# NathanBWaters/playaid_core

Hardware: AMD Instinct MI355X
Metric: 1080p frames/sec end-to-end (higher is better)
Workload: dtype f32; 1 GPU; configs[1]: 64 x 1080x1920 BGR frames per GPU per clip; parallelism=single GPU, lanes=2, ingest=raw BGR frames resident in HBM

## Files before the change

playaid_core_amd/csrc/igemm.hip:

```cpp
#include "tile_common.h"
#include <cstdio>
#include <cstdlib>

namespace pa {

#ifndef PA_COUNTED_VMCNT
#define PA_COUNTED_VMCNT 0
#endif

template <int BM, int BN, int BK, bool GATHER, int ABL = 0, bool SKIPW = false>
__global__ __launch_bounds__(256) void igemm_f32_kernel(const GemmParams p) {
    constexpr int MI = BM / 64;
    constexpr int NI = BN / 64;
    using Stage = Im2colStage<4, BK, BM, BN, GATHER>;
    constexpr int LDS_STRIDE = BK;
    constexpr int A_ROWS = Stage::A_ROWS, B_ROWS = Stage::B_ROWS;
    constexpr int STAGE = (BM + BN) * LDS_STRIDE;
    __shared__ __attribute__((aligned(16))) float lds[3 * STAGE];

    Stage st;
    st.setup(p);
    const int tile_m = st.tile_m, tile_n = st.tile_n, z = st.z;
    const int ks_begin = st.ks_begin, ks_end = st.ks_end;
    const int tid = threadIdx.x;
    const int wave_id = __builtin_amdgcn_readfirstlane(tid >> 6);
#define PA_ISSUE_STAGE(BUF)                                                \
    {                                                                      \
        float* As_w = lds + (BUF) * STAGE + wave_id * 256;                 \
        st.issue(p, As_w, As_w + BM * LDS_STRIDE);                         \
    }

    const int lane = tid & 63;
    const int wave = tid >> 6;
    const int wm = wave >> 1, wn = wave & 1;
    const int lr = lane & 31;
    const int lh = lane >> 5;
// ... 222 lines not shown
    plan_splitk(p.ktot / bk, p.splitk, p.ksteps_per_split);
    hipError_t err;
    switch (tile) {
        case TILE_128x128: err = launch_tile<128, 128, 32>(p, s); break;
        case TILE_128x64: err = launch_tile<128, 64, 32>(p, s); break;
        case TILE_64x64: err = launch_tile<64, 64, 32>(p, s); break;
        case TILE_128x64_K64: err = launch_tile<128, 64, 64>(p, s); break;
        default: err = launch_tile<64, 64, 64>(p, s); break;
    }
    if (err != hipSuccess) return err;
    if (p.splitk_used) *p.splitk_used = p.splitk;
    if (p.splitk > 1 && !p.defer_reduce) return launch_splitk_reduce(p, s);
    return hipSuccess;
}

hipError_t launch_splitk_reduce(const GemmParams& p, hipStream_t s, bool out_bf16) {
    const size_t total = (size_t)p.M * (p.N >> 2);
    int grid = (int)((total + 255) / 256);
    if (grid > 2048) grid = 2048;
    if (out_bf16) hipLaunchKernelGGL(splitk_reduce_kernel<bf16_t>, dim3(grid), dim3(256), 0, s, p);
    else hipLaunchKernelGGL(splitk_reduce_kernel<float>, dim3(grid), dim3(256), 0, s, p);
    return hipGetLastError();
}

}
```

playaid_core_amd/csrc/misc.hip:

```cpp
#include "tile_common.h"
#include "../../include/playaid_hip.h"

namespace pa {

__global__ __launch_bounds__(256) void nchw_to_padded_kernel(const float* __restrict__ x, float* __restrict__ out, int n, int out_bf16) {
    const size_t total = (size_t)n * 128 * 128;
    for (size_t i = (size_t)blockIdx.x * blockDim.x + threadIdx.x; i < total; i += (size_t)gridDim.x * blockDim.x) {
        const int img = (int)(i >> 14);
        const int pix = (int)(i & 16383);
        const int y = pix >> 7, xx = pix & 127;
        const float* s = x + (size_t)img * 3 * 16384 + pix;
        float4 v;
        v.x = s[0];
        v.y = s[16384];
        v.z = s[32768];
        v.w = 0.f;
        const size_t o = ((size_t)img * 134 + (y + 3)) * 134 + (xx + 3);
        if (out_bf16) {
            reinterpret_cast<uint2*>(out)[o] = make_uint2(pack_bf16x2(v.x, v.y), f32_to_bf16(v.z));
        } else {
            reinterpret_cast<float4*>(out)[o] = v;
        }
    }
}
// ... 115 lines not shown
        sum.x *= 0.0625f;
        sum.y *= 0.0625f;
        sum.z *= 0.0625f;
        sum.w *= 0.0625f;
        reinterpret_cast<float4*>(out)[i] = sum;
    }
}

hipError_t launch_avgpool(const float* in, float* out, int32_t n, hipStream_t s) {
    const size_t total = (size_t)n * 128;
    const int grid = (int)((total + 255) / 256);
    hipLaunchKernelGGL(avgpool_kernel, dim3(grid), dim3(256), 0, s, in, out, n);
    return hipGetLastError();
}

__global__ void window_gather_kernel(int32_t* gather, int frame_num_lo, int count, int fighters, int seq, int delta,
                                     int max_frames, int min_frame, int sub_frames) {
    const int i = blockIdx.x * blockDim.x + threadIdx.x;
    const int total = count * fighters * seq;
    if (i >= total) return;
    const int t = i % seq;
    const int w = i / seq;
    const int fighter = w % fighters;
    const int f = frame_num_lo + w / fighters;
    if (sub_frames > 0) {
        const int c = (f - 1) / sub_frames;
        min_frame = c * sub_frames + 1;
        max_frames = (c + 1) * sub_frames;
    }
    const int mid = seq / 2;
// ... 182 lines not shown
```

playaid_core_amd/csrc/pa_api.hip:

```cpp
#include "../../include/playaid_hip.h"
#include "conv_rows.h"

#include <algorithm>
#include <cmath>
#include <cstdio>
#include <cstdlib>
#include <cstring>
#include <string>
#include <vector>

using namespace pa;

namespace {

constexpr int WINO_TICKETS = 4096;

struct ConvLayer {
    std::string name;
    int cin, cout, kh, kw, stride;
    int in_hw, out_hw;
    int in_pad, out_pad;
    int off;
    int taps, kw_taps, chunk;
    int in_px_stride;
// ... 3 lines not shown
    float* wgt = nullptr;
    float* wino_wgt = nullptr;
    int wino_bn = 0;
    float* bias = nullptr;
    int relu = 1;
    GemmTile tile = TILE_128x64;
    int splitk = 1;
    bool forced = false;
    float* in2 = nullptr;
    int in2_c = 0, in2_hw = 0, in2_stride = 1;
    float* ds_wgt = nullptr;
    float* ds_out = nullptr;
    float* ds_next_wgt = nullptr;
    float* ds_next_out = nullptr;
    std::string ds_next_name;
    bool ds_fused = false;
    bool ds_probe = false;
    double k_alg = 0;
    unsigned short* split_wgt = nullptr;
    unsigned short* ds_split_wgt = nullptr;
};

struct ProfEntry {
    int name_id;
    hipEvent_t start, stop;
    double flops, bytes;
    double flops_executed;
};

}
// ... 24 lines not shown
    float* x0 = nullptr;
    float* x0_slot[2] = {nullptr, nullptr};
    int32_t* pre_status[2] = {nullptr, nullptr};
    float* pooled = nullptr;
    float* feats_tmp = nullptr;
    float* cache = nullptr;
    int32_t* cache_status = nullptr;
    float* h1 = nullptr;
    int32_t* gather = nullptr;
    int gather_key[4] = {-1, -1, -1, -1};
    float* slab = nullptr;
    size_t slab_floats = 0;
    float* wino_tickets = nullptr;
    std::vector<ConvLayer> convs;
    ConvLayer fc;
    float* stem_wgt_bf16 = nullptr;
    float* c1 = nullptr;
    float* p1 = nullptr;
    float* layer4_out = nullptr;
    float* w1d = nullptr;
    float* b1d = nullptr;
    float *w2 = nullptr, *b2 = nullptr, *w3 = nullptr, *b3 = nullptr;
    GemmTile head_tile = TILE_64x64;
    int head_splitk = 16;
    CropPlan* plans = nullptr;
    int32_t* coef = nullptr;
    int coef_dim = 0;
    int32_t* coef_cache = nullptr;
    int coef_cache_pad = -1, coef_cache_dmax = 0;
    AreaTabPacked* area_tabs = nullptr;
// ... 275 lines not shown
        p.k2_steps = L.in2_c / (bf ? 64 : 32);
        p.in2_px_stride = L.in2_c;
        p.in2_row_stride = w2 * L.in2_c;
        p.in2_img_stride = w2 * w2 * L.in2_c;
        p.stride2 = L.in2_stride;
        p.off2 = 1;
        p.ktot += L.in2_c;
    }
    GemmTile tile = L.tile;
    int splitk = L.splitk;
    if (!L.forced) choose_tile(p.M, p.N, p.ktot / (bf ? 64 : 32), &tile, &splitk);
    p.splitk = splitk;
    const size_t slab_avail = e->slab_floats > slab_off ? e->slab_floats - slab_off : 0;
    if ((size_t)p.splitk * p.M * p.N > slab_avail) p.splitk = 1;
    const bool f32_branch = !bf && !e->emu && L.ds_next_wgt;
    const bool f32_branch_here = f32_branch && p.splitk <= 1;
    const bool ds_here = (bf && L.ds_next_wgt) || f32_branch_here;
    if (bf && L.ds_next_wgt) {
        p.wgt2 = L.ds_next_wgt;
        p.out2 = at(L.ds_next_out, crop0 * out_crop);
    }
    if ((bf && L.ds_next_wgt) || (bf && L.ds_probe)) {
        tile = (p.N % 128 == 0 && ((p.M + 127) / 128) * (p.N / 128) >= 256) ? TILE_128x128 : TILE_128x64;
        p.splitk = 1;
    }
    const double k_main = ((bf_ds || f32_ds) ? L.k_alg - L.in2_c : L.k_alg) + (ds_here ? L.cin : 0);
    const double flops = 2.0 * p.M * p.N * k_main;
    const double bytes = (double)es * ((double)ncrops * L.in_hw * L.in_hw * L.cin + (double)p.M * p.N * ((L.residual || bf_ds || f32_ds || ds_here) ? 2 : 1) +
                                       (double)p.N * k_main + ((L.in2 && !bf_ds && !f32_ds) ? (double)ncrops * L.in2_hw * L.in2_hw * L.in2_c : 0.0));
    const bool as_wino = !bf && L.wino_wgt && !p.act2;
    bool branch_left = f32_branch;
    {
// ... 29 lines not shown
            if (pe == hipErrorInvalidValue) pe = launch_igemm(p, tile, s);
            HIPCHK(e, pe);
        } else {
            static const int use_pgemm = getenv("PA_S2_PGEMM") ? atoi(getenv("PA_S2_PGEMM")) : 2;
            hipError_t pe = hipErrorInvalidValue;
            const bool pg = use_pgemm && L.kh == 3 && L.stride == 2 && !p.act2 && !p.residual && p.splitk <= 1 && !p.gather;
            if (pg && f32_branch_here) {
                p.wgt2 = L.ds_next_wgt;
                p.out2 = at(L.ds_next_out, crop0 * out_crop);
                pe = launch_pgemm(p, 64, s);
                if (pe == hipSuccess) branch_left = false;
                p.wgt2 = nullptr;
                p.out2 = nullptr;
            }
            if (pg && pe == hipErrorInvalidValue) pe = launch_pgemm(p, use_pgemm == 2 ? 64 : 0, s);
            if (pe == hipErrorInvalidValue) pe = launch_igemm(p, tile, s);
            HIPCHK(e, pe);
        }
    }
    if (branch_left) {
        const GemmParams d = branch_gemm_of(L.in, L.in_hw, L.cin, L.stride, L.ds_next_wgt, L.ds_next_out);
        ProfScope ps(e, s, e->profile_layers ? L.ds_next_name.c_str() : prof_name, 2.0 * d.M * d.N * L.cin,
                     4.0 * ((double)ncrops * L.in_hw * L.in_hw * L.cin / (L.stride * L.stride) + (double)d.M * d.N + (double)d.N * L.cin));
        HIPCHK(e, launch_f32_branch(d));
    }
    return PA_OK;
}

int run_backbone_part(pa_engine* e, int crop0, int ncrops, const float* x_in, float* feats_out, size_t slab_off, hipStream_t s,
                      int stop = PA_TRACE_STAGES) {
    int rc;
    ConvLayer stem = e->convs[0];
    stem.in = const_cast<float*>(x_in);
    static const bool stem_igemm = getenv("PA_STEM_IGEMM") && atoi(getenv("PA_STEM_IGEMM"));
    auto stem_part = [&](int c0, int n, hipStream_t st) -> int {
        if (stem_igemm && !e->bf16) return run_conv(e, stem, c0, n, slab_off, st, "igemm_conv7x7_stem");
        StemParams sp;
        memset(&sp, 0, sizeof(sp));
        sp.x = x_in + (size_t)c0 * 134 * 134 * 4;
// ... 62 lines not shown
                if ((rc = run_conv(e, Nx, crop0, ncrops, slab_off, e->side, "igemm_conv1x1_ds", true))) return rc;
                HIPCHK(e, hipEventRecord(e->ev_ds_join, e->side));
                ds_pending = true;
            }
        }
        const bool use_pending = ds_pending && L.in2 && L.ds_wgt && L.wino_wgt;
        if (use_pending) HIPCHK(e, hipStreamWaitEvent(s, e->ev_ds_join, 0));
        rc = run_conv(e, L, crop0, ncrops, slab_off, s, pn, false, use_pending);
        if (use_pending) ds_pending = false;
        if (rc) return rc;
        if (stop <= (int)i + 1) {
            if (ds_pending) HIPCHK(e, hipStreamWaitEvent(s, e->ev_ds_join, 0));
            return PA_OK;
        }
    }
    {
        ProfScope ps(e, s, "avgpool", 0.0, ncrops * ((e->bf16 ? 2.0 : 4.0) * 16.0 * 512 + 4.0 * 512));
        if (e->bf16)
            HIPCHK(e, launch_avgpool_bf16(reinterpret_cast<uint16_t*>(e->layer4_out) + (size_t)crop0 * 36 * 512,
                                          e->pooled + (size_t)crop0 * 512, ncrops, s));
        else
            HIPCHK(e, launch_avgpool(e->layer4_out + (size_t)crop0 * 36 * 512, e->pooled + (size_t)crop0 * 512, ncrops, s));
    }
    if (stop <= 18) return PA_OK;
    ConvLayer fc = e->fc;
    fc.out = feats_out;
    rc = run_conv(e, fc, crop0, ncrops, slab_off, s, "igemm_fc");
    return rc;
}

// ... 202 lines not shown
    ALLOC(e->c1, (size_t)NC * 66 * 66 * 64, true);
    ALLOC(e->p1, (size_t)NC * 34 * 34 * 64, true);
    ALLOC(e->pooled, (size_t)NC * 512, true);
    ALLOC(e->feats_tmp, (size_t)NC * PA_FEATURE_STRIDE, true);
    ALLOC(e->jpeg_qtab, 128, true);
    ALLOC(e->crops_tmp, (size_t)NC * PA_CROP * PA_CROP * 3, true);
    ALLOC(e->cache, (size_t)e->cache_rows * PA_FEATURE_STRIDE, true);
    ALLOC(e->cache_status, (size_t)e->cache_rows, true);
    ALLOC(e->h1, (size_t)NC * 512, true);
    ALLOC(e->gather, (size_t)NC * S, true);
    ALLOC(e->status_tmp, (size_t)NC, true);
    ALLOC(e->dev_errors, 4, true);
    e->clean_g6_cap = (size_t)cfg->max_clip_frames * 8 * 6;
    ALLOC(e->clean_g6, e->clean_g6_cap, false);

    e->arena_cap = pa_weight_blob_bytes(S, A) / 4 * 13 + (1u << 20);
    {
        void* ar = nullptr;
        HIPCHK(e, hipMalloc(&ar, e->arena_cap));
        e->allocs.push_back(ar);
        e->arena = reinterpret_cast<uint8_t*>(ar);
    }
    if (!e->adopt) e->arena_stage.assign(e->arena_cap, 0);
    static const float dry_source[1] = {0.f};
    const float* blob_f = e->adopt ? dry_source : reinterpret_cast<const float*>(hdr + 8);
    BlobReader br{blob_f, 0, blob_float_count(S, A), e->adopt};
    std::vector<float> keep_w, keep_b;
    auto add_conv = [&](const std::string& name, int cin, int cout, int k, int stride, int in_hw, float* in, float* outb,
                        float* residual, int relu, bool keep = false) -> int {
        ConvLayer L;
        L.name = name;
// ... 115 lines not shown
                    static const int wino_min_hw = getenv("PA_WINO_MIN_HW") ? atoi(getenv("PA_WINO_MIN_HW")) : 4;
                    if (wino_mode && wino_ds && hw_out >= wino_min_hw && hw_out % 4 == 0) {
                        L.wino_bn = wino_pick_bn(co, (long long)NC * (hw_out / 4) * (hw_out / 4), co);
                        std::vector<float> ug(wino_weight_floats(co, co), 0.f);
                        if (!br.dry) wino_transform_weights(keep_w.data(), co, co, L.wino_bn, ug.data());
                        rc = upload(e, &L.wino_wgt, ug);
                        if (rc) return rc;
                        rc = upload(e, &L.ds_wgt, wd);
                        if (rc) return rc;
                        if (e->emu && (rc = upload_split(e, &L.ds_split_wgt, wd, co, cin, false))) return rc;
                        ALLOC(L.ds_out, buf, true);
                        static const int f32_ds_fuse = getenv("PA_F32_DS_FUSE") ? atoi(getenv("PA_F32_DS_FUSE")) : 1;
                        static const int ds_side_knob = getenv("PA_DS_SIDE") ? atoi(getenv("PA_DS_SIDE")) : 0;
                        static const int s2_pgemm_knob = getenv("PA_S2_PGEMM") ? atoi(getenv("PA_S2_PGEMM")) : 2;
                        ConvLayer& C1 = e->convs[e->convs.size() - 2];
                        if (f32_ds_fuse && !ds_side_knob && s2_pgemm_knob && !e->emu && li < 3 && C1.in == cur && C1.kh == 3 &&
                            C1.stride == 2 && C1.cout == co && C1.out_hw == hw_out && C1.out_pad == L.out_pad && C1.chunk == cin && C1.cin == cin &&
                            C1.in_hw == hw_in[li] && C1.in_pad == 1 && !C1.forced) {
                            C1.ds_next_wgt = L.ds_wgt;
                            C1.ds_next_out = L.ds_out;
                            C1.ds_next_name = L.name;
                            L.ds_fused = true;
                        }
                    }
                }
                rc = upload(e, &L.bias, bf);
                if (rc) return rc;
                L.in2 = cur;
                L.in2_c = cin;
                L.in2_hw = hw_in[li];
                L.in2_stride = stride;
                L.k_alg += cin;
            }
            rc = add_conv(pre + ".1.conv1", co, co, 3, 1, hw_out, outA, mid, nullptr, 1);
            if (rc) return rc;
            rc = add_conv(pre + ".1.conv2", co, co, 3, 1, hw_out, mid, outB, outA, 1);
// ... 11 lines not shown
        if (!br.dry) {
            memcpy(wp.data(), w, sizeof(float) * 1000 * 512);
            memcpy(bp.data(), b, sizeof(float) * 1000);
        }
        ConvLayer& L = e->fc;
        L.name = "fc";
        L.cin = 512; L.cout = PA_FEATURE_STRIDE; L.kh = L.kw = 1; L.stride = 1;
        L.in_hw = 1; L.out_hw = 1; L.in_pad = 0; L.out_pad = 0; L.off = 0;
        L.taps = 1; L.kw_taps = 1; L.chunk = 512; L.in_px_stride = 512;
        L.in = e->pooled; L.out = nullptr; L.residual = nullptr; L.relu = 0;
        L.k_alg = 512.0 * 1000.0 / 1024.0;
        rc = upload(e, &L.wgt, wp);
        if (rc) return rc;
        rc = upload(e, &L.bias, bp);
        if (rc) return rc;
        L.tile = TILE_64x64;
        L.splitk = 4;
        L.forced = true;
        if (const char* fs = getenv("PA_FC_SPLITK")) L.splitk = std::max(1, atoi(fs));
    }
    {
        const float* w = br.take((size_t)512 * 1000 * S);
        const float* b = br.take(512);
        if (!w || !b) return fail(e, PA_ERR_BAD_WEIGHTS, "weight blob too short at cnn1d");
        std::vector<float> wp((size_t)512 * S * PA_FEATURE_STRIDE, 0.f);
        for (int o = 0; o < 512 && !br.dry; ++o)
            for (int c = 0; c < 1000; ++c)
                for (int t = 0; t < S; ++t)
                    wp[((size_t)o * S + t) * PA_FEATURE_STRIDE + c] = w[((size_t)o * 1000 + c) * S + t];
        rc = upload(e, &e->w1d, wp);
// ... 169 lines not shown
        bytes = n * w * w * L.cout * es;
        has_branch = L.in2 != nullptr;
        aux_src = L.ds_out;
    } else if (stage == 18) {
        src = e->pooled;
        bytes = n * 512 * sizeof(float);
    } else {
        src = e->feats_tmp;
        bytes = n * PA_FEATURE_STRIDE * sizeof(float);
    }
    if (out_bytes < bytes) return fail(e, PA_ERR_INVALID_ARG, "pa_backbone_trace: out is smaller than the stage");
    if (has_branch && aux) {
        if (!aux_src) return fail(e, PA_ERR_INVALID_ARG, "pa_backbone_trace: this stage stores no downsample branch");
        if (aux_bytes < bytes) return fail(e, PA_ERR_INVALID_ARG, "pa_backbone_trace: aux is smaller than the stage");
    }
    hipStream_t s = (hipStream_t)stream;
    HIPCHK(e, launch_nchw_to_padded(x, e->x0, n_crops, e->bf16 ? 1 : 0, s));
    if (stage > 0) {
        const int rc = run_backbone(e, n_crops, e->x0, e->feats_tmp, s, stage);
        if (rc) return rc;
    }
    HIPCHK(e, hipMemcpyAsync(out, src, bytes, hipMemcpyDeviceToDevice, s));
    if (has_branch && aux) HIPCHK(e, hipMemcpyAsync(aux, aux_src, bytes, hipMemcpyDeviceToDevice, s));
    return PA_OK;
}

int pa_crop_resize_width(pa_engine* e, const uint8_t* frames, int32_t n, int32_t height, int32_t width, const int32_t* rects_host,
                         int32_t n_rects, int32_t out_w, uint8_t* out, int32_t out_h_cap, int32_t* out_h_host, void* stream) {
    if (!e || !frames || !rects_host || !out || !out_h_host || n < 1 || height < 1 || width < 1 || n_rects < 1 || n_rects > 4 || out_w < 1 ||
        out_h_cap < 1)
        return fail(e, PA_ERR_INVALID_ARG, "pa_crop_resize_width: bad argument");
    RectResizeParams q;
    memset(&q, 0, sizeof(q));
    q.frames = frames;
    q.height = height;
    q.width = width;
    q.n_rects = n_rects;
    q.out_w = out_w;
// ... 248 lines not shown
    hipStream_t s = (hipStream_t)stream;
    const int F = e->cfg.num_fighters;
    HIPCHK(e, hipMemcpyAsync(e->cache_status + (size_t)frame0 * F, e->pre_status[slot], sizeof(int32_t) * n * F,
                             hipMemcpyDeviceToDevice, s));
    int rc = run_backbone(e, n * F, e->x0_slot[slot], e->cache + (size_t)frame0 * F * PA_FEATURE_STRIDE, s);
    if (rc) return rc;
    for (int i = 0; i < n; ++i) e->ready[frame0 + i] = 1;
    return PA_OK;
}

int pa_backbone_frames(pa_engine* e, const uint8_t* frames, int32_t n, int32_t height, int32_t width, const double* boxes,
                       int32_t frame0, uint8_t* crops_rgb, int32_t* status, void* stream) {
    if (!e || frame0 < 0) return fail(e, PA_ERR_INVALID_ARG, "pa_backbone_frames: bad argument");
    if (e->clip_frames < 1) return fail(e, PA_ERR_INVALID_ARG, "pa_backbone_frames: call pa_clip_begin first");
    if (frame0 + n > e->clip_frames) return fail(e, PA_ERR_CAPACITY, "pa_backbone_frames: frames exceed clip capacity");
    int rc = pa_preprocess_frames(e, frames, n, height, width, boxes, 0, crops_rgb, status, stream);
    if (rc) return rc;
    return pa_backbone_slot(e, 0, n, frame0, stream);
}

int pa_backbone_frames_indexed(pa_engine* e, const uint8_t* frames, int32_t n, int32_t height, int32_t width,
                               const double* boxes, const int32_t* frame_ids, uint8_t* crops_rgb, int32_t* status, void* stream) {
    if (!e || !frame_ids) return fail(e, PA_ERR_INVALID_ARG, "pa_backbone_frames_indexed: bad argument");
    if (e->clip_frames < 1) return fail(e, PA_ERR_INVALID_ARG, "pa_backbone_frames_indexed: call pa_clip_begin first");
    int rc = pa_preprocess_frames(e, frames, n, height, width, boxes, 0, crops_rgb, status, stream);
    if (rc) return rc;
    hipStream_t s = (hipStream_t)stream;
    const int F = e->cfg.num_fighters;
    rc = run_backbone(e, n * F, e->x0_slot[0], e->feats_tmp, s);
    if (rc) return rc;
    ProfScope ps(e, s, "scatter_features", 0.0, 2.0 * n * F * PA_FEATURE_STRIDE * 4.0);
    HIPCHK(e, launch_scatter_rows(e->feats_tmp, e->pre_status[0], frame_ids, e->cache, e->cache_status, n, F, e->clip_frames,
                                  e->dev_errors, s));
// ... 472 lines not shown
```

playaid_core_amd/csrc/pa_kernels.h:

```cpp
#pragma once
#include <hip/hip_runtime.h>
#include <stdint.h>

namespace pa {

__device__ __forceinline__ float silu_fast(float x) {
    return x * __builtin_amdgcn_rcpf(1.0f + __builtin_amdgcn_exp2f(x * -1.44269504088896341f));
}

struct GemmParams {
    const float* act;
    const float* wgt;
    const float* bias;
    const float* residual;
    float* out;
    float* slab;
    const int32_t* gather;
    int32_t M, N, ktot;
    int32_t taps, kw_taps, chunk;
    int32_t howo, wo;
    int32_t howo_shift, wo_shift;
    int32_t in_img_stride, in_row_stride, in_px_stride, stride, off_y, off_x;
    int32_t out_img_stride, out_row_stride, out_px_stride, out_pad;
    int32_t relu;
// ... 11 lines not shown
    int32_t up_img_stride, up_row_stride, up_px_stride, up_pad;
    int32_t patch_slots, patch_pitch, img_px, tiles_per_img, p0_img, p0_row, total_px;
    int32_t swz_a, magic_pitch, magic_img, img_px_patch;
    int32_t xcd_m, xcd_n;
    int32_t blk_rows, blk_cols, blk_shift_c, blk_shift_px, blk_per_row, blk_per_img, n_blocks, src_pitch;
    const float* wgt2;
    float* out2;
    unsigned long long* clk;
    int32_t* tickets;
};

enum GemmTile { TILE_128x128 = 0, TILE_128x64 = 1, TILE_64x64 = 2, TILE_128x64_K64 = 3, TILE_64x64_K64 = 4,
                TILE_256x128 = 5  };

hipError_t launch_igemm(const GemmParams& p, GemmTile tile, hipStream_t s);
hipError_t launch_pgemm(const GemmParams& p, int bm, hipStream_t s);
int psgemm_pick_bn(int N, int residual);
size_t psgemm_weight_elems(int N, int ktot, int residual);
void psgemm_pack_weights(const float* w, int N, int ktot, int residual, unsigned short* out);
hipError_t launch_psgemm(const GemmParams& p, const unsigned short* wsp, size_t out_floats, size_t up_floats, hipStream_t s);
size_t bgemm_weight_elems(int N, int ktot, int residual);
void bgemm_pack_weights(const float* w, int N, int ktot, int residual, unsigned short* out);
hipError_t launch_bgemm(const GemmParams& p, const unsigned short* wsp, size_t out_elems, size_t up_elems, bool out_f32, hipStream_t s);
constexpr int BGEMM_SLAB_ITEMS = 256, BGEMM_TICKETS = 4 * 128, BGEMM_SPLIT_MAX_GRID = 64, BGEMM_SPLIT_MIN_KSTEPS = 72;
int bgemm_pick_split(const GemmParams& p, int force);
hipError_t launch_igemm_bf16(const GemmParams& p, GemmTile tile, hipStream_t s);

hipError_t launch_conv3x3_bf16_patch(const GemmParams& p, hipStream_t s);

struct StemParams {
// ... 210 lines not shown
    float img_w, img_h;
    float* dets;
    int32_t* counts;
};
hipError_t launch_detect_nms(const DetectParams& q, hipStream_t s);
constexpr int DETECT_MAX_CLASSES = 80;
hipError_t launch_detect_nms_classes(const DetectParams& q, hipStream_t s);

hipError_t launch_linear_f32(const float* X, int ld, const float* W, const float* bias, float* C, int ldc, int M, int N, int K, int relu,
                             hipStream_t s);
hipError_t launch_spin(int32_t microseconds, hipStream_t s);
hipError_t launch_gate(const int* flag, int32_t max_microseconds, hipStream_t s);
hipError_t launch_nchw_to_padded(const float* x, float* out, int32_t n, int32_t out_bf16, hipStream_t s);
hipError_t launch_maxpool(const float* in, float* out, int32_t n, hipStream_t s);
hipError_t launch_avgpool(const float* in, float* out, int32_t n, hipStream_t s);
hipError_t launch_maxpool_bf16(const void* in, void* out, int32_t n, hipStream_t s);
hipError_t launch_avgpool_bf16(const void* in, float* out, int32_t n, hipStream_t s);
hipError_t launch_window_gather(int32_t* gather, int32_t frame_num_lo, int32_t count, int32_t fighters,
                                int32_t seq, int32_t delta, int32_t max_frames, int32_t min_frame, int32_t sub_frames, hipStream_t s);
hipError_t launch_identity_gather(int32_t* gather, int32_t n, hipStream_t s);
hipError_t launch_scatter_rows(const float* feats, const int32_t* st, const int32_t* ids, float* cache, int32_t* cache_st,
                               int32_t n, int32_t fighters, int32_t clip_frames, int32_t* bad_ids, hipStream_t s);

struct HeadParams {
    const float* h1;
    const float* slab;
    const float* b1;
    int32_t splitk;
    const float* w2;
    const float* b2;
// ... 29 lines not shown
```

playaid_core_amd/csrc/tile_common.h:

```cpp
#pragma once
#include "pa_kernels.h"

namespace pa {


typedef float f32x16 __attribute__((ext_vector_type(16)));
typedef float f32x4 __attribute__((ext_vector_type(4)));
typedef float f32x2 __attribute__((ext_vector_type(2)));
typedef uint32_t u32x4 __attribute__((ext_vector_type(4)));
typedef __bf16 bf16x8 __attribute__((ext_vector_type(8)));
typedef uint16_t bf16_t;

__device__ __forceinline__ int xcd_remap(int b, int nwg) {
    const int q = nwg >> 3, r = nwg & 7, xcd = b & 7;
    return (xcd < r ? xcd * (q + 1) : r * (q + 1) + (xcd - r) * q) + (b >> 3);
}

__device__ __forceinline__ void xcd_grid_tile(int xcd, int rank, int gm, int gn, int tiles_m, int tiles_n, int& tile_m, int& tile_n) {
    const int tm_per = tiles_m / gm, tn_per = tiles_n / gn;
    const int xm = xcd / gn, lm = rank / tn_per;
    tile_m = xm * tm_per + lm;
    tile_n = (xcd - xm * gn) * tn_per + (rank - lm * tn_per);
}

// ... 55 lines not shown
struct Im2colStage {
    static constexpr int CH = BK * EB / 16;
    static constexpr int PASS_ROWS = 256 / CH;
    static constexpr int A_ROWS = BM / PASS_ROWS;
    static constexpr int B_ROWS = BN / PASS_ROWS;
    static constexpr int CE = 16 / EB;

    int z, tile_m, tile_n;
    int row0, colq;
    int a_off[A_ROWS], a_off2[A_ROWS], b_off[B_ROWS];
    int nk_main, ks_begin, ks_end;
    int issue_ks;
    int cur_kc, cur_kx, cur_ky;
    __amdgpu_buffer_rsrc_t act_rs, wgt_rs, act2_rs;

    __device__ __forceinline__ void setup(const GemmParams& p) {
        const int wg = xcd_remap(blockIdx.x, gridDim.x);
        const int tiles_mn = p.tiles_m * p.tiles_n;
        z = wg / tiles_mn;
        const int t_id = wg - z * tiles_mn;
        tile_m = t_id / p.tiles_n;
        tile_n = t_id - tile_m * p.tiles_n;

        const int tid = threadIdx.x;
        row0 = tid / CH;
        colq = (tid & (CH - 1)) ^ (CH == 8 ? ((row0 >> 1) & 7) : (row0 & 15));
#pragma unroll
        for (int i = 0; i < A_ROWS; ++i) {
            int m = tile_m * BM + row0 + PASS_ROWS * i;
            m = m < p.M ? m : p.M - 1;
            a_off2[i] = 0;
            if (GATHER) {
// ... 124 lines not shown
```

playaid_core_amd/engine.py:

```python
from __future__ import annotations

import ctypes as C
from typing import Dict, List, Mapping, Optional, Tuple

import numpy as np
import torch

from . import _lib, constants
from .weights import infer_geometry, pack_state_dict


class EngineError(RuntimeError):
    def __init__(self, code: int, msg: str):
        super().__init__(f"playaid_hip error {code}: {msg}")
        self.code = code


def _ptr(t: Optional[torch.Tensor]):
    return C.c_void_p(t.data_ptr()) if t is not None else C.c_void_p(0)


class WeightsArena:

    def __init__(self, data: torch.Tensor, sequence_length: int, num_actions: int, compute_dtype: str):
# ... 153 lines not shown
        if stage == 1:
            return (n, 34, 34, 64)
        if 2 <= stage <= 17:
            li = (stage - 2) // 4
            hw = (32, 16, 8, 4)[li] + 2
            return (n, hw, hw, (64, 128, 256, 512)[li])
        if stage == 18:
            return (n, 512)
        if stage == 19:
            return (n, _lib.PA_FEATURE_STRIDE)
        raise ValueError(f"stage must be 0..{_lib.PA_TRACE_STAGES - 1}")

    def backbone_trace(self, x: torch.Tensor, stage: int, aux: bool = False):
        if x.dim() != 4 or tuple(x.shape[1:]) != (3, 128, 128):
            raise ValueError(f"expected [n,3,128,128], got {tuple(x.shape)}")
        if aux and stage not in self.TRACE_BRANCH_STAGES:
            raise ValueError(f"aux exists at stages {self.TRACE_BRANCH_STAGES} only")
        xd = self._dev(x, torch.float32)
        n = xd.shape[0]
        dt = torch.bfloat16 if self.compute_dtype == "bf16" and stage <= 17 else torch.float32
        out = torch.empty(self.trace_shape(n, stage), dtype=dt, device=self.device)
        br = torch.empty_like(out) if aux else None
        nbytes = out.numel() * out.element_size()
        self._check(self._lib.pa_backbone_trace(self._h, _ptr(xd), n, stage, _ptr(out), nbytes, _ptr(br),
                                                nbytes if aux else 0, self._stream()))
        return (out, br) if aux else out

    def crop_resize_width(self, frames, rects, out_w: int = 256):
        fd = self._dev(frames, torch.uint8)
        n, h, w, _ = fd.shape
        rects = [tuple(int(v) for v in r) for r in rects]
        if not 1 <= len(rects) <= 4:
            raise ValueError("1..4 rectangles per call")
        cap = 1
        for (x1, y1, x2, y2) in rects:
            if x2 > x1 and y2 > y1:
                cap = max(cap, int((y2 - y1) * (out_w / float(x2 - x1))))
        out = torch.zeros((n, len(rects), cap, out_w, 3), dtype=torch.uint8, device=self.device)
        flat = (C.c_int32 * (4 * len(rects)))(*[v for r in rects for v in r])
        oh = (C.c_int32 * len(rects))()
# ... 468 lines not shown
```

Baseline: 64220 frames/s.

## Fuse avgpool with FC, group downsample GEMM, write status directly

Adds a pool_fc kernel that fuses the 4x4 average pool with the 512->1024 FC layer, using weights repacked on the host at load time so the pool and FC no longer run as separate launches. It also adds a grouped igemm launch that runs a split-K stride-2 3x3 conv and its 1x1 downsample branch in a single grid, which is now enabled for layer4 as well. Finally, pa_backbone_frames preprocesses straight into the cache status and backbone, skipping the intermediate slot path. Together these cut kernel launches and intermediate traffic, at the cost of more code paths, a larger weight arena and new validation constraints.

```diff
diff --git a/playaid_core_amd/csrc/igemm.hip b/playaid_core_amd/csrc/igemm.hip
--- a/playaid_core_amd/csrc/igemm.hip
+++ b/playaid_core_amd/csrc/igemm.hip
@@ -8,8 +8,10 @@
 #define PA_COUNTED_VMCNT 0
 #endif
 
-template <int BM, int BN, int BK, bool GATHER, int ABL = 0, bool SKIPW = false>
-__global__ __launch_bounds__(256) void igemm_f32_kernel(const GemmParams p) {
+template <int BM, int BN, int BK, bool GATHER, int ABL = 0, bool SKIPW = false, class... Second>
+__global__ __launch_bounds__(256) void igemm_f32_kernel(GemmParams p, const Second... second) {
+    constexpr bool GROUPED = sizeof...(Second) == 1;
+    static_assert(sizeof...(Second) <= 1, "one second GEMM at most");
     constexpr int MI = BM / 64;
     constexpr int NI = BN / 64;
     using Stage = Im2colStage<4, BK, BM, BN, GATHER>;
@@ -19,7 +21,19 @@
     __shared__ __attribute__((aligned(16))) float lds[3 * STAGE];
 
     Stage st;
-    st.setup(p);
+    if constexpr (GROUPED) {
+        const int own = p.tiles_m * p.tiles_n * p.splitk;
+        int wg;
+        if ((int)blockIdx.x >= own) {
+            wg = xcd_remap(blockIdx.x - own, gridDim.x - own);
+            p = (second, ...);
+        } else {
+            wg = xcd_remap(blockIdx.x, own);
+        }
+        st.setup(p, wg);
+    } else {
+        st.setup(p);
+    }
     const int tile_m = st.tile_m, tile_n = st.tile_n, z = st.z;
     const int ks_begin = st.ks_begin, ks_end = st.ks_end;
     const int tid = threadIdx.x;
@@ -272,6 +286,34 @@
     return hipSuccess;
 }
 
+hipError_t launch_igemm_grouped(const GemmParams& p_in, const GemmParams& g_in, GemmTile tile, hipStream_t s) {
+    if (tile != TILE_64x64 && tile != TILE_128x64) return hipErrorInvalidValue;
+    struct { GemmParams p, g; } a;
+    a.p = p_in;
+    a.g = g_in;
+    const TileDims d = tile_dims(tile, 4);
+    for (GemmParams* q : {&a.p, &a.g}) {
+        if (q->N % d.bn != 0 || q->chunk % d.bk != 0 || q->ktot != q->taps * q->chunk || q->k2_steps || q->gather || q->skip_w || q->M <= 0)
+            return hipErrorInvalidValue;
+        fill_pow2_shifts(*q);
+        q->tiles_m = (q->M + d.bm - 1) / d.bm;
+        q->tiles_n = q->N / d.bn;
+    }
+    plan_splitk(a.p.ktot / d.bk, a.p.splitk, a.p.ksteps_per_split);
+    a.g.splitk = 1;
+    plan_splitk(a.g.ktot / d.bk, a.g.splitk, a.g.ksteps_per_split);
+    if (a.p.splitk <= 1 || a.p.defer_reduce) return hipErrorInvalidValue;
+    const int grid = a.p.tiles_m * a.p.tiles_n * a.p.splitk + a.g.tiles_m * a.g.tiles_n;
+    if (tile == TILE_64x64)
+        hipLaunchKernelGGL((igemm_f32_kernel<64, 64, 32, false, 0, false, GemmParams>), dim3(grid), dim3(256), 0, s, a.p, a.g);
+    else
+        hipLaunchKernelGGL((igemm_f32_kernel<128, 64, 32, false, 0, false, GemmParams>), dim3(grid), dim3(256), 0, s, a.p, a.g);
+    hipError_t err = hipGetLastError();
+    if (err != hipSuccess) return err;
+    if (a.p.splitk_used) *a.p.splitk_used = a.p.splitk;
+    return launch_splitk_reduce(a.p, s);
+}
+
 hipError_t launch_splitk_reduce(const GemmParams& p, hipStream_t s, bool out_bf16) {
     const size_t total = (size_t)p.M * (p.N >> 2);
     int grid = (int)((total + 255) / 256);
diff --git a/playaid_core_amd/csrc/misc.hip b/playaid_core_amd/csrc/misc.hip
--- a/playaid_core_amd/csrc/misc.hip
+++ b/playaid_core_amd/csrc/misc.hip
@@ -153,6 +153,118 @@
     return hipGetLastError();
 }
 
+constexpr int PF_ROWS = 4, PF_COLS = 128, PF_K = 512, PF_N = 1024, PF_NK = PF_K / 32, PF_GROUPS = 4;
+static_assert(PF_ROWS == 4 && PF_COLS * 4 == PF_K, "a float4 of crops per k; 128 threads pool one crop's 512 channels");
+typedef float pf_f32x2 __attribute__((ext_vector_type(2)));
+
+template <int CHUNK>
+__global__ __launch_bounds__(PF_COLS * PF_GROUPS) void pool_fc_kernel(const float* __restrict__ in, const float* __restrict__ wgt_kq,
+                                                                      const float* __restrict__ bias, float* __restrict__ pooled,
+                                                                      float* __restrict__ out, int out_stride, int n, int splitk, int per) {
+    __shared__ __attribute__((aligned(16))) float lds[PF_K * PF_ROWS + PF_NK * PF_ROWS * PF_COLS];
+    float* const a_s = lds;
+    float* const part = lds + PF_K * PF_ROWS;
+    const int item = xcd_remap(blockIdx.x, gridDim.x);
+    const int tile_n = item % (PF_N / PF_COLS), tile_m = item / (PF_N / PF_COLS);
+    const int t = threadIdx.x & (PF_COLS - 1), g = threadIdx.x / PF_COLS;
+    const int row0 = tile_m * PF_ROWS;
+    const int col = tile_n * PF_COLS + t;
+    const float4* w4 = reinterpret_cast<const float4*>(wgt_kq) + col;
+
+    float4 wv[CHUNK * 8];
+    if (g < splitk) {
+#pragma unroll
+        for (int i = 0; i < CHUNK * 8; ++i) wv[i] = w4[(size_t)(g * per * 8 + i) * PF_N];
+    }
+    {
+        float4 sum = make_float4(0.f, 0.f, 0.f, 0.f);
+        if (row0 + g < n) {
+            const float4* src = reinterpret_cast<const float4*>(in) + (size_t)(row0 + g) * 36 * 128 + t;
+#pragma unroll
+            for (int y = 1; y <= 4; ++y)
+#pragma unroll
+                for (int x = 1; x <= 4; ++x) {
+                    const float4 v = src[(size_t)(y * 6 + x) * 128];
+                    sum.x += v.x;
+                    sum.y += v.y;
+                    sum.z += v.z;
+                    sum.w += v.w;
+                }
+            sum.x *= 0.0625f;
+            sum.y *= 0.0625f;
+            sum.z *= 0.0625f;
+            sum.w *= 0.0625f;
+            if (tile_n == 0) reinterpret_cast<float4*>(pooled)[(size_t)(row0 + g) * 128 + t] = sum;
+        }
+        a_s[(4 * t + 0) * PF_ROWS + g] = sum.x;
+        a_s[(4 * t + 1) * PF_ROWS + g] = sum.y;
+        a_s[(4 * t + 2) * PF_ROWS + g] = sum.z;
+        a_s[(4 * t + 3) * PF_ROWS + g] = sum.w;
+    }
+    __syncthreads();
+
+    for (int z = g; z < splitk; z += PF_GROUPS) {
+        const int ks0 = z * per, ks1 = ks0 + per < PF_NK ? ks0 + per : PF_NK;
+        pf_f32x2 acc01 = {0.f, 0.f}, acc23 = {0.f, 0.f};
+        for (int ks = ks0; ks < ks1; ks += CHUNK) {
+            if (ks != g * per) {
+#pragma unroll
+                for (int i = 0; i < CHUNK * 8; ++i) wv[i] = w4[(size_t)(ks * 8 + i) * PF_N];
+            }
+#pragma unroll
+            for (int kk = 0; kk < CHUNK * 4; ++kk) {
+                const float4 w_lo = wv[2 * kk], w_hi = wv[2 * kk + 1];
+                const float wlo[4] = {w_lo.x, w_lo.y, w_lo.z, w_lo.w}, whi[4] = {w_hi.x, w_hi.y, w_hi.z, w_hi.w};
+                const float* a_k = a_s + (size_t)(ks * 32 + kk * 8) * PF_ROWS;
+#pragma unroll
+                for (int j = 0; j < 4; ++j) {
+                    const float4 alo = *reinterpret_cast<const float4*>(a_k + j * PF_ROWS);
+                    const float4 ahi = *reinterpret_cast<const float4*>(a_k + (4 + j) * PF_ROWS);
+                    acc01 = __builtin_elementwise_fma(pf_f32x2{alo.x, alo.y}, pf_f32x2{wlo[j], wlo[j]}, acc01);
+                    acc23 = __builtin_elementwise_fma(pf_f32x2{alo.z, alo.w}, pf_f32x2{wlo[j], wlo[j]}, acc23);
+                    acc01 = __builtin_elementwise_fma(pf_f32x2{ahi.x, ahi.y}, pf_f32x2{whi[j], whi[j]}, acc01);
+                    acc23 = __builtin_elementwise_fma(pf_f32x2{ahi.z, ahi.w}, pf_f32x2{whi[j], whi[j]}, acc23);
+                }
+            }
+        }
+        float* dst = part + (size_t)z * PF_ROWS * PF_COLS + t;
+        dst[0 * PF_COLS] = acc01.x;
+        dst[1 * PF_COLS] = acc01.y;
+        dst[2 * PF_COLS] = acc23.x;
+        dst[3 * PF_COLS] = acc23.y;
+    }
+    __syncthreads();
+
+    if (row0 + g < n) {
+        const float* src = part + g * PF_COLS + t;
+        float s = src[0];
+        for (int z = 1; z < splitk; ++z) s += src[(size_t)z * PF_ROWS * PF_COLS];
+        const float b = bias[col];
+        s += splitk > 1 ? b : b + 0.f;
+        out[(size_t)(row0 + g) * out_stride + col] = s;
+    }
+}
+
+void pool_fc_pack_weights(const float* w, float* out) {
+    for (int kq = 0; kq < PF_K / 4; ++kq)
+        for (int c = 0; c < PF_N; ++c)
+            for (int j = 0; j < 4; ++j) out[((size_t)kq * PF_N + c) * 4 + j] = w[(size_t)c * PF_K + kq * 4 + j];
+}
+
+hipError_t launch_pool_fc(const float* in, const float* wgt_kq, const float* bias, float* pooled, float* out, int32_t out_stride, int32_t n,
+                          int32_t splitk, int32_t ksteps_per_split, hipStream_t s) {
+    if (n < 1 || splitk < 1 || ksteps_per_split < 1 || (splitk - 1) * ksteps_per_split >= PF_NK || splitk * ksteps_per_split < PF_NK)
+        return hipErrorInvalidValue;
+    const int grid = ((n + PF_ROWS - 1) / PF_ROWS) * (PF_N / PF_COLS);
+    if (ksteps_per_split % 4 == 0)
+        hipLaunchKernelGGL(pool_fc_kernel<4>, dim3(grid), dim3(PF_COLS * PF_GROUPS), 0, s, in, wgt_kq, bias, pooled, out, out_stride, n, splitk,
+                           ksteps_per_split);
+    else
+        hipLaunchKernelGGL(pool_fc_kernel<1>, dim3(grid), dim3(PF_COLS * PF_GROUPS), 0, s, in, wgt_kq, bias, pooled, out, out_stride, n, splitk,
+                           ksteps_per_split);
+    return hipGetLastError();
+}
+
 __global__ void window_gather_kernel(int32_t* gather, int frame_num_lo, int count, int fighters, int seq, int delta,
                                      int max_frames, int min_frame, int sub_frames) {
     const int i = blockIdx.x * blockDim.x + threadIdx.x;
diff --git a/playaid_core_amd/csrc/pa_api.hip b/playaid_core_amd/csrc/pa_api.hip
--- a/playaid_core_amd/csrc/pa_api.hip
+++ b/playaid_core_amd/csrc/pa_api.hip
@@ -1,5 +1,6 @@
 #include "../../include/playaid_hip.h"
 #include "conv_rows.h"
+#include "tile_common.h"
 
 #include <algorithm>
 #include <cmath>
@@ -41,6 +42,7 @@
     float* ds_next_wgt = nullptr;
     float* ds_next_out = nullptr;
     std::string ds_next_name;
+    bool ds_next_split_only = false;
     bool ds_fused = false;
     bool ds_probe = false;
     double k_alg = 0;
@@ -95,6 +97,7 @@
     float* wino_tickets = nullptr;
     std::vector<ConvLayer> convs;
     ConvLayer fc;
+    float* fc_wgt_kq = nullptr;
     float* stem_wgt_bf16 = nullptr;
     float* c1 = nullptr;
     float* p1 = nullptr;
@@ -400,8 +403,19 @@
     const size_t slab_avail = e->slab_floats > slab_off ? e->slab_floats - slab_off : 0;
     if ((size_t)p.splitk * p.M * p.N > slab_avail) p.splitk = 1;
     const bool f32_branch = !bf && !e->emu && L.ds_next_wgt;
-    const bool f32_branch_here = f32_branch && p.splitk <= 1;
-    const bool ds_here = (bf && L.ds_next_wgt) || f32_branch_here;
+    const bool f32_branch_here = f32_branch && p.splitk <= 1 && !L.ds_next_split_only;
+    static const int ds_group = getenv("PA_F32_DS_GROUP") ? atoi(getenv("PA_F32_DS_GROUP")) : 1;
+    bool ds_grouped = false;
+    if (ds_group && f32_branch && p.splitk > 1 && L.kh == 3 && L.stride == 2 && !p.act2 && !p.residual && !(L.wino_wgt && !p.act2) &&
+        (tile == TILE_64x64 || tile == TILE_128x64)) {
+        GemmTile dt;
+        int dsk;
+        choose_tile(p.M, p.N, L.cin / 32, &dt, &dsk);
+        int32_t sk = p.splitk, per = 0;
+        plan_splitk(p.ktot / 32, sk, per);
+        ds_grouped = dt == tile && sk > 1;
+    }
+    const bool ds_here = (bf && L.ds_next_wgt) || f32_branch_here || ds_grouped;
     if (bf && L.ds_next_wgt) {
         p.wgt2 = L.ds_next_wgt;
         p.out2 = at(L.ds_next_out, crop0 * out_crop);
@@ -461,6 +475,10 @@
                 p.out2 = nullptr;
             }
             if (pg && pe == hipErrorInvalidValue) pe = launch_pgemm(p, use_pgemm == 2 ? 64 : 0, s);
+            if (ds_grouped && pe == hipErrorInvalidValue) {
+                pe = launch_igemm_grouped(p, branch_gemm_of(L.in, L.in_hw, L.cin, L.stride, L.ds_next_wgt, L.ds_next_out), tile, s);
+                if (pe == hipSuccess) branch_left = false;
+            }
             if (pe == hipErrorInvalidValue) pe = launch_igemm(p, tile, s);
             HIPCHK(e, pe);
         }
@@ -470,6 +488,8 @@
         ProfScope ps(e, s, e->profile_layers ? L.ds_next_name.c_str() : prof_name, 2.0 * d.M * d.N * L.cin,
                      4.0 * ((double)ncrops * L.in_hw * L.in_hw * L.cin / (L.stride * L.stride) + (double)d.M * d.N + (double)d.N * L.cin));
         HIPCHK(e, launch_f32_branch(d));
+    } else if (ds_grouped && e->profiling) {
+        ProfScope ps(e, s, e->profile_layers ? L.ds_next_name.c_str() : prof_name, 0.0, 0.0);
     }
     return PA_OK;
 }
@@ -562,6 +582,24 @@
             return PA_OK;
         }
     }
+    static const int pool_fc = getenv("PA_POOL_FC") ? atoi(getenv("PA_POOL_FC")) : 1;
+    if (pool_fc && stop > 18 && !e->bf16 && e->fc_wgt_kq && !e->fc.split_wgt && e->fc.chunk == 512 && e->fc.cout == PA_FEATURE_STRIDE) {
+        const ConvLayer& fc = e->fc;
+        GemmTile tile = fc.tile;
+        int splitk = fc.splitk;
+        if (!fc.forced) choose_tile(ncrops, fc.cout, fc.chunk / 32, &tile, &splitk);
+        const size_t slab_avail = e->slab_floats > slab_off ? e->slab_floats - slab_off : 0;
+        if ((size_t)splitk * ncrops * fc.cout > slab_avail) splitk = 1;
+        if (tile_dims(tile, 4).bk == 32) {
+            int32_t sk = splitk, per = 0;
+            plan_splitk(fc.chunk / 32, sk, per);
+            ProfScope ps(e, s, "pool_fc", 2.0 * ncrops * fc.cout * fc.k_alg,
+                         4.0 * ((double)ncrops * 16.0 * 512 + (double)ncrops * 512 + (double)ncrops * fc.cout + (double)fc.cout * fc.k_alg));
+            HIPCHK(e, launch_pool_fc(e->layer4_out + (size_t)crop0 * 36 * 512, e->fc_wgt_kq, fc.bias, e->pooled + (size_t)crop0 * 512,
+                                     feats_out + (size_t)crop0 * fc.cout, fc.cout, ncrops, sk, per, s));
+            return PA_OK;
+        }
+    }
     {
         ProfScope ps(e, s, "avgpool", 0.0, ncrops * ((e->bf16 ? 2.0 : 4.0) * 16.0 * 512 + 4.0 * 512));
         if (e->bf16)
@@ -794,7 +832,7 @@
     e->clean_g6_cap = (size_t)cfg->max_clip_frames * 8 * 6;
     ALLOC(e->clean_g6, e->clean_g6_cap, false);
 
-    e->arena_cap = pa_weight_blob_bytes(S, A) / 4 * 13 + (1u << 20);
+    e->arena_cap = pa_weight_blob_bytes(S, A) / 4 * 13 + (3u << 20);
     {
         void* ar = nullptr;
         HIPCHK(e, hipMalloc(&ar, e->arena_cap));
@@ -940,12 +978,14 @@
                         static const int ds_side_knob = getenv("PA_DS_SIDE") ? atoi(getenv("PA_DS_SIDE")) : 0;
                         static const int s2_pgemm_knob = getenv("PA_S2_PGEMM") ? atoi(getenv("PA_S2_PGEMM")) : 2;
                         ConvLayer& C1 = e->convs[e->convs.size() - 2];
-                        if (f32_ds_fuse && !ds_side_knob && s2_pgemm_knob && !e->emu && li < 3 && C1.in == cur && C1.kh == 3 &&
+                        static const int ds_group_knob = getenv("PA_F32_DS_GROUP") ? atoi(getenv("PA_F32_DS_GROUP")) : 1;
+                        if (f32_ds_fuse && !ds_side_knob && s2_pgemm_knob && !e->emu && (li < 3 || ds_group_knob) && C1.in == cur && C1.kh == 3 &&
                             C1.stride == 2 && C1.cout == co && C1.out_hw == hw_out && C1.out_pad == L.out_pad && C1.chunk == cin && C1.cin == cin &&
                             C1.in_hw == hw_in[li] && C1.in_pad == 1 && !C1.forced) {
                             C1.ds_next_wgt = L.ds_wgt;
                             C1.ds_next_out = L.ds_out;
                             C1.ds_next_name = L.name;
+                            C1.ds_next_split_only = li == 3;
                             L.ds_fused = true;
                         }
                     }
@@ -987,6 +1027,12 @@
         if (rc) return rc;
         rc = upload(e, &L.bias, bp);
         if (rc) return rc;
+        if (!e->bf16) {
+            std::vector<float> wq(wp.size(), 0.f);
+            if (!br.dry) pool_fc_pack_weights(wp.data(), wq.data());
+            rc = upload(e, &e->fc_wgt_kq, wq);
+            if (rc) return rc;
+        }
         L.tile = TILE_64x64;
         L.splitk = 4;
         L.forced = true;
@@ -1186,6 +1232,8 @@
         if (!aux_src) return fail(e, PA_ERR_INVALID_ARG, "pa_backbone_trace: this stage stores no downsample branch");
         if (aux_bytes < bytes) return fail(e, PA_ERR_INVALID_ARG, "pa_backbone_trace: aux is smaller than the stage");
     }
+    const size_t pooled_bytes = n * 512 * sizeof(float);
+    if (stage == 19 && aux && aux_bytes < pooled_bytes) return fail(e, PA_ERR_INVALID_ARG, "pa_backbone_trace: aux is smaller than the pooled features");
     hipStream_t s = (hipStream_t)stream;
     HIPCHK(e, launch_nchw_to_padded(x, e->x0, n_crops, e->bf16 ? 1 : 0, s));
     if (stage > 0) {
@@ -1194,6 +1242,7 @@
     }
     HIPCHK(e, hipMemcpyAsync(out, src, bytes, hipMemcpyDeviceToDevice, s));
     if (has_branch && aux) HIPCHK(e, hipMemcpyAsync(aux, aux_src, bytes, hipMemcpyDeviceToDevice, s));
+    if (stage == 19 && aux) HIPCHK(e, hipMemcpyAsync(aux, e->pooled, pooled_bytes, hipMemcpyDeviceToDevice, s));
     return PA_OK;
 }
 
@@ -1472,9 +1521,25 @@
     if (!e || frame0 < 0) return fail(e, PA_ERR_INVALID_ARG, "pa_backbone_frames: bad argument");
     if (e->clip_frames < 1) return fail(e, PA_ERR_INVALID_ARG, "pa_backbone_frames: call pa_clip_begin first");
     if (frame0 + n > e->clip_frames) return fail(e, PA_ERR_CAPACITY, "pa_backbone_frames: frames exceed clip capacity");
-    int rc = pa_preprocess_frames(e, frames, n, height, width, boxes, 0, crops_rgb, status, stream);
+    static const int status_direct = getenv("PA_STATUS_DIRECT") ? atoi(getenv("PA_STATUS_DIRECT")) : 1;
+    if (!status_direct) {
+        int rc = pa_preprocess_frames(e, frames, n, height, width, boxes, 0, crops_rgb, status, stream);
+        if (rc) return rc;
+        return pa_backbone_slot(e, 0, n, frame0, stream);
+    }
+    if (!frames || !boxes || n < 1 || height < 1 || width < 1) return fail(e, PA_ERR_INVALID_ARG, "pa_preprocess_frames: bad argument");
+    if (n > e->cfg.max_batch_frames || height > e->cfg.max_frame_height || width > e->cfg.max_frame_width)
+        return fail(e, PA_ERR_CAPACITY, "pa_preprocess_frames: frames exceed engine capacity");
+    hipStream_t s = (hipStream_t)stream;
+    const int F = e->cfg.num_fighters;
+    int32_t* st = e->cache_status + (size_t)frame0 * F;
+    int rc = run_preprocess(e, frames, n, height, width, boxes, e->cfg.crop_padding, 1, crops_rgb, e->x0_slot[0], st, s);
     if (rc) return rc;
-    return pa_backbone_slot(e, 0, n, frame0, stream);
+    if (status) HIPCHK(e, hipMemcpyAsync(status, st, sizeof(int32_t) * n * F, hipMemcpyDeviceToDevice, s));
+    rc = run_backbone(e, n * F, e->x0_slot[0], e->cache + (size_t)frame0 * F * PA_FEATURE_STRIDE, s);
+    if (rc) return rc;
+    for (int i = 0; i < n; ++i) e->ready[frame0 + i] = 1;
+    return PA_OK;
 }
 
 int pa_backbone_frames_indexed(pa_engine* e, const uint8_t* frames, int32_t n, int32_t height, int32_t width,
diff --git a/playaid_core_amd/csrc/pa_kernels.h b/playaid_core_amd/csrc/pa_kernels.h
--- a/playaid_core_amd/csrc/pa_kernels.h
+++ b/playaid_core_amd/csrc/pa_kernels.h
@@ -49,6 +49,7 @@
                 TILE_256x128 = 5  };
 
 hipError_t launch_igemm(const GemmParams& p, GemmTile tile, hipStream_t s);
+hipError_t launch_igemm_grouped(const GemmParams& p, const GemmParams& g, GemmTile tile, hipStream_t s);
 hipError_t launch_pgemm(const GemmParams& p, int bm, hipStream_t s);
 int psgemm_pick_bn(int N, int residual);
 size_t psgemm_weight_elems(int N, int ktot, int residual);
@@ -289,6 +290,9 @@
 hipError_t launch_nchw_to_padded(const float* x, float* out, int32_t n, int32_t out_bf16, hipStream_t s);
 hipError_t launch_maxpool(const float* in, float* out, int32_t n, hipStream_t s);
 hipError_t launch_avgpool(const float* in, float* out, int32_t n, hipStream_t s);
+void pool_fc_pack_weights(const float* w, float* out);
+hipError_t launch_pool_fc(const float* in, const float* wgt_kq, const float* bias, float* pooled, float* out, int32_t out_stride, int32_t n,
+                          int32_t splitk, int32_t ksteps_per_split, hipStream_t s);
 hipError_t launch_maxpool_bf16(const void* in, void* out, int32_t n, hipStream_t s);
 hipError_t launch_avgpool_bf16(const void* in, float* out, int32_t n, hipStream_t s);
 hipError_t launch_window_gather(int32_t* gather, int32_t frame_num_lo, int32_t count, int32_t fighters,
diff --git a/playaid_core_amd/csrc/tile_common.h b/playaid_core_amd/csrc/tile_common.h
--- a/playaid_core_amd/csrc/tile_common.h
+++ b/playaid_core_amd/csrc/tile_common.h
@@ -93,8 +93,8 @@
     int cur_kc, cur_kx, cur_ky;
     __amdgpu_buffer_rsrc_t act_rs, wgt_rs, act2_rs;
 
-    __device__ __forceinline__ void setup(const GemmParams& p) {
-        const int wg = xcd_remap(blockIdx.x, gridDim.x);
+    __device__ __forceinline__ void setup(const GemmParams& p) { setup(p, xcd_remap(blockIdx.x, gridDim.x)); }
+    __device__ __forceinline__ void setup(const GemmParams& p, int wg) {
         const int tiles_mn = p.tiles_m * p.tiles_n;
         z = wg / tiles_mn;
         const int t_id = wg - z * tiles_mn;
diff --git a/playaid_core_amd/engine.py b/playaid_core_amd/engine.py
--- a/playaid_core_amd/engine.py
+++ b/playaid_core_amd/engine.py
@@ -191,16 +191,16 @@
     def backbone_trace(self, x: torch.Tensor, stage: int, aux: bool = False):
         if x.dim() != 4 or tuple(x.shape[1:]) != (3, 128, 128):
             raise ValueError(f"expected [n,3,128,128], got {tuple(x.shape)}")
-        if aux and stage not in self.TRACE_BRANCH_STAGES:
-            raise ValueError(f"aux exists at stages {self.TRACE_BRANCH_STAGES} only")
+        if aux and stage not in self.TRACE_BRANCH_STAGES and stage != 19:
+            raise ValueError(f"aux exists at stages {self.TRACE_BRANCH_STAGES} and 19 only")
         xd = self._dev(x, torch.float32)
         n = xd.shape[0]
         dt = torch.bfloat16 if self.compute_dtype == "bf16" and stage <= 17 else torch.float32
         out = torch.empty(self.trace_shape(n, stage), dtype=dt, device=self.device)
-        br = torch.empty_like(out) if aux else None
+        br = (torch.empty((n, 512), dtype=torch.float32, device=self.device) if stage == 19 else torch.empty_like(out)) if aux else None
         nbytes = out.numel() * out.element_size()
         self._check(self._lib.pa_backbone_trace(self._h, _ptr(xd), n, stage, _ptr(out), nbytes, _ptr(br),
-                                                nbytes if aux else 0, self._stream()))
+                                                br.numel() * br.element_size() if aux else 0, self._stream()))
         return (out, br) if aux else out
 
     def crop_resize_width(self, frames, rects, out_w: int = 256):
```

After: 64730 frames/s, median of 6. No clear change (+0.8%).
